# ProjectTorreyPines/TorJ.jl

Measured on AMD Instinct MI355X. Metric: ray-steps/sec, 1e5-ray EC fan on 1 MI355X (+ 2/4/8-GPU scaling), higher is better.
Workload: dtype f64

## Files before the change

### torj.jl_amd/csrc/torj_args.hpp

```cpp
#pragma once
#include "torj_math.hpp"

struct TraceArgs {
    const double *coef;
    const double *cellp;
    Grid g;
    Consts k;
    double omega;
    int mode;
    double ds;
    int n_steps;
    int chunk_steps;
    double psi_exit;
    double P_min;
    int n;
    const double *x0;
    const double *N0;
    const double *w;
    double *state;
    int *status;
    int *steps;
    int n_psi;
    const double *grid;
    double *dP;
// ... 11 lines not shown
    double abstol, reltol, s_step;
    int n_chunks;
    int *chunk;
    int n_hist, hist_off;
};

constexpr int kTsLds = 7 * 7 * 64;

constexpr int kDepoNone = 0, kDepoBinned = 1, kDepoSamples = 2;

#ifndef TORJ_BLOCK
#define TORJ_BLOCK 256
#endif
#ifndef TORJ_MIN_WAVES
#define TORJ_MIN_WAVES 2
#endif
#ifndef TORJ_GROUP
#define TORJ_GROUP 64
#endif
#ifndef TORJ_WARM_MIN_WAVES
#define TORJ_WARM_MIN_WAVES 1
#endif

constexpr int kAinF = 5;
constexpr int kAinFW = 6;

struct SplitArgs {
    double *ain;
    double *alpha;
    unsigned *awork;
    double *psib;
    double *cbx;
    double *tx;
    int *tinfo;
    double *stau, *spsi, *sPdep;
    int *sinfo;
    unsigned char *zflag;
    double zval;
    int k0, kb;
    int nf;
    int tile_cap;
    double tile_margin;
    int traj_mode;
    int nan_step;
    unsigned long long *defer;
    unsigned *defer_cnt;
    int defer_lrm;
    int zlatch;
};

constexpr int kSplitMaxSteps = 1 << 24;
__device__ __forceinline__ int info_steps(int v) { return v & 0xffffff; }
__device__ __forceinline__ int info_status(int v) { return (unsigned)v >> 24; }
__device__ __forceinline__ int make_info(int steps, int st) { return steps | (st << 24); }

#ifndef TORJ_AIN_TRAJ_MATH
#define TORJ_AIN_TRAJ_MATH 0
#endif
#ifndef TORJ_TRAJ_WAVES
#define TORJ_TRAJ_WAVES TORJ_MIN_WAVES
#endif
#ifndef TORJ_ALPHA_WAVES
#define TORJ_ALPHA_WAVES 6
#endif
#ifndef TORJ_ALPHA_UNROLL
#define TORJ_ALPHA_UNROLL 1
#endif
#ifndef TORJ_TILE_NODES
#define TORJ_TILE_NODES 256
#endif
constexpr int kTileNodes = TORJ_TILE_NODES;
#ifndef TORJ_TILE_CELLS
// ... 39 lines not shown
```

### torj.jl_amd/csrc/torj_k_alpha.hpp

```cpp
#pragma once
#include "torj_args.hpp"
#include "torj_k_fused.hpp"
#include "torj_warm.hpp"

#ifndef TORJ_ALPHA_BLOCK
#define TORJ_ALPHA_BLOCK 128
#endif
constexpr int kAlphaBlock = TORJ_ALPHA_BLOCK;
#ifndef TORJ_ALPHA_SETPRIO
#define TORJ_ALPHA_SETPRIO 0
#endif
template <bool COUNT>
__global__ void __launch_bounds__(kAlphaBlock, TORJ_ALPHA_WAVES) k_alpha_pts(TraceArgs a, SplitArgs sp, int nq) {
#if TORJ_ALPHA_SETPRIO
    __builtin_amdgcn_s_setprio(TORJ_ALPHA_SETPRIO);
#endif
    const int q = blockIdx.x, js = blockIdx.y;
    const int i = q * kAlphaBlock + threadIdx.x;
    if (i >= a.n) return;
    const int j = js >> 2;
    const int ti = sp.tinfo[i], si = sp.sinfo[i];
    const int zf = sp.zflag ? sp.zflag[i] : 0;
    if (__all(zf != 0)) {
#if defined(TORJ_ALPHA_PROF) && defined(__HIP_DEVICE_COMPILE__)
        TORJ_APROF_WAVE(kAprofZ);
#endif
        sp.alpha[(size_t)js * a.n + i] = sp.zval;
        if constexpr (COUNT) sp.awork[(size_t)js * a.n + i] = 0u;
        return;
    }
    const double *in = sp.ain + (size_t)js * sp.nf * a.n + i;
    const double X = in[0], Y = in[(size_t)a.n], N2 = in[2 * (size_t)a.n], Npar = in[3 * (size_t)a.n];
    const double lnTe = in[4 * (size_t)a.n];
    asm volatile("" ::"v"(ti), "v"(si), "v"(X), "v"(Y), "v"(N2), "v"(Npar), "v"(lnTe));
    if (sp.k0 + j >= info_steps(ti) || info_status(si) != ST_OK) return;
#if defined(TORJ_ALPHA_PROF) && defined(__HIP_DEVICE_COMPILE__)
    {
        const unsigned long long am = __ballot(1), zm = __ballot(zf != 0);
        if ((int)__lane_id() == __builtin_ffsll((long long)am) - 1) {
            atomicAdd(&g_aprof[4], 1ull);
            atomicAdd(&g_aprof[5], (unsigned long long)__popcll(am));
            atomicAdd(&g_aprof[14], (unsigned long long)__popcll(zm));
        }
    }
#endif
    const double Nabs = TORJ_AIN_TRAJ_MATH ? N2 : sqrt_pos(N2), Te = TORJ_AIN_TRAJ_MATH ? lnTe : exp_fast<true>(lnTe);
    if constexpr (COUNT) {
        AlbajarWork work = {};
        sp.alpha[(size_t)js * a.n + i] = abs_albajar_fast_body<1, TORJ_ALPHA_UNROLL>(
            c_gl, a.omega, X, Y, Nabs, Npar, Te, a.mode, &work, 0, c_gl.tiny_alpha);
        sp.awork[(size_t)js * a.n + i] = (work.n_active & 1u) | ((work.n_harm & 3u) << 1) |
                                     ((work.n_zero & 3u) << 3) | (min(work.n_terms, 2047u) << 5) |
                                     ((work.n_negl & 3u) << 16) | ((work.n_early & 3u) << 18);
    } else {
        sp.alpha[(size_t)js * a.n + i] = abs_albajar_fast_body<1, TORJ_ALPHA_UNROLL>(
            c_gl, a.omega, X, Y, Nabs, Npar, Te, a.mode, nullptr, 0, c_gl.tiny_alpha);
    }
}

#ifndef TORJ_ALPHA_PPW
#define TORJ_ALPHA_PPW 1
#endif
#ifndef TORJ_ALPHA_PREFETCH
#define TORJ_ALPHA_PREFETCH 1
#endif
template <bool COUNT, int P>
__global__ void __launch_bounds__(kAlphaBlock, TORJ_ALPHA_WAVES) k_alpha_pts_mp(TraceArgs a, SplitArgs sp, int nq) {
    const int i = blockIdx.x * kAlphaBlock + threadIdx.x;
    if (i >= a.n) return;
    const int js0 = blockIdx.y * P;
    const int np = min(P, 4 * sp.kb - js0);
    const int ti = sp.tinfo[i], si = sp.sinfo[i];
    const int js_end = info_status(si) != ST_OK ? 0 : 4 * (info_steps(ti) - sp.k0);
    const size_t n = (size_t)a.n, stride = (size_t)sp.nf * n;
    const double *in = sp.ain + (size_t)js0 * stride + i;
    double X = in[0], Y = in[n], N2 = in[2 * n], Npar = in[3 * n], lnTe = in[4 * n];
    for (int p = 0; p < np; p++) {
        const int js = js0 + p;
        const GLTable *glp = &c_gl;
        asm volatile("" : "+s"(glp));
#if TORJ_ALPHA_PREFETCH
        double Xn = 0.0, Yn = 0.0, N2n = 0.0, Nparn = 0.0, lnTen = 0.0;
        if (p + 1 < np) {
            const double *nx = in + (size_t)(p + 1) * stride;
            Xn = nx[0], Yn = nx[n], N2n = nx[2 * n], Nparn = nx[3 * n], lnTen = nx[4 * n];
        }
#endif
        if (js < js_end) {
            const double Nabs = TORJ_AIN_TRAJ_MATH ? N2 : sqrt_pos(N2),
                         Te = TORJ_AIN_TRAJ_MATH ? lnTe : exp_fast<true>(lnTe);
            if constexpr (COUNT) {
// ... 96 lines not shown
```

### torj.jl_amd/csrc/torj_k_scan.hpp

```cpp
#pragma once
#include "torj_args.hpp"
#include "torj_k_fused.hpp"
#include "torj_k_traj.hpp"

__device__ void cold_replay(const TraceArgs &a, const SplitArgs &sp, int i, double x[3], double N[3], int k) {
    const TileCell cg{a.cellp, nullptr, 0, 0, 0, 0};
    const TileCoef ng{a.coef, nullptr, 0, 0, 0, 0};
    ZBox zb;
    for (int s = 0; s < k; s++) {
        double xn[3], Nn[3], psi;
        double *o_run = ain_row(a, sp, 0, i);
        if (sp.traj_mode == kTrajCell)
            cold_step<true, kTileNS, TileCell, true>(a, cg, sp, 0, i, x, N, xn, Nn, &psi, zb, false, o_run);
        else if (sp.traj_mode == kTrajTile)
            cold_step<true, kTileNS, TileCoef, true>(a, ng, sp, 0, i, x, N, xn, Nn, &psi, zb, false, o_run);
        else
            cold_step<true, kNF, const double *, true>(a, a.coef, sp, 0, i, x, N, xn, Nn, &psi, zb, false, o_run);
#pragma unroll
        for (int c = 0; c < 3; c++) {
            x[c] = xn[c];
            N[c] = Nn[c];
        }
    }
}

template <int DEPO, bool TRAJ, bool COUNT>
__device__ __forceinline__ void tau_scan_body(const TraceArgs &a, const SplitArgs &sp) {
    const int i = blockIdx.x * 64 + threadIdx.x;
    unsigned long long nsteps = 0, c2 = 0, c3 = 0, c4 = 0, c5 = 0, c6 = 0, c7 = 0;
    const int am = a.abs_model;
    if (i < a.n) {
        int steps = 0, st = ST_OK;
        double tau = 0.0, psi_a = 0.0, Pdep = 0.0;
        if (sp.k0 > 0) {
            const int v = sp.sinfo[i];
            steps = info_steps(v);
            st = info_status(v);
            tau = sp.stau[i];
            Pdep = sp.sPdep[i];
        }
        if constexpr (DEPO == kDepoBinned) psi_a = sp.spsi[i];
        if (st == ST_OK) {
            const int tv = sp.tinfo[i];
            const int tT = info_steps(tv), tS = info_status(tv);
            const double w = (DEPO == kDepoBinned && a.w) ? a.w[i] : 1.0;
            const double ds6 = a.ds / 6.0;
            double P = exp(-tau);
            DepoAcc dacc = {-1, 0.0};
            const int s_end = min(a.n_steps, sp.k0 + sp.kb);
            constexpr int kScanBatch = 4;
            bool done = false;
            for (int sb = steps; sb < s_end && !done; sb += kScanBatch) {
                double alb[kScanBatch][4];
#pragma unroll
                for (int v = 0; v < kScanBatch; v++) {
                    const size_t ov = (size_t)(min(sb + v, s_end - 1) - sp.k0) * 4 * a.n + i;
#pragma unroll
                    for (int q = 0; q < 4; q++) alb[v][q] = sp.alpha[ov + q * (size_t)a.n];
                }
#pragma unroll
                for (int v = 0; v < kScanBatch; v++) {
                    const int s = sb + v;
                    if (s >= s_end) break;
                    if (s >= tT) {
                        if (tS == ST_NAN) st = ST_NAN;
                        done = true;
                        break;
                    }
                    const size_t o = (size_t)(s - sp.k0) * 4 * a.n + i;
                    const double al0 = (s == sp.nan_step && i % 3 == 0) ? (double)NAN : alb[v][0];
                    const double al1 = alb[v][1], al2 = alb[v][2], al3 = alb[v][3];
                    double acc_a = fma(1.0, al0, 0.0);
                    acc_a = fma(2.0, al1, acc_a);
                    acc_a = fma(2.0, al2, acc_a);
                    acc_a = fma(1.0, al3, acc_a);
                    const double taun = tau + ds6 * acc_a;
                    if (!isfinite(taun)) {
                        st = ST_NAN | 0x40;
                        done = true;
                        break;
                    }
#pragma unroll
                    for (int q = 0; q < 4 && COUNT; q++) {
                        const unsigned wk = sp.awork[o + q * (size_t)a.n];
                        if (am == 1) {
                            c2 += wk & 1u;
                            c3 += (wk >> 1) & 3u;
                            c5 += (wk >> 3) & 3u;
                            c4 += (wk >> 5) & 2047u;
                            c6 += (wk >> 16) & 3u;
                            c7 += (wk >> 18) & 3u;
                        } else if (am == 2) {
                            const unsigned lrm = wk >> 21, passes = (wk >> 14) & 127u;
                            c2 += wk & 127u;
                            c3 += (wk >> 7) & 127u;
                            c4 += passes;
                            c5 += passes * lrm;
                            c6 += lrm;
                            c7 += lrm * lrm;
                        }
                    }
                    const double Pn = exp(-taun);
                    const double dP = P - Pn;
                    if constexpr (DEPO == kDepoSamples) {
                        if (s > 0) a.smp_dpds[smp_at(s, i, a.smp_rows)] = P * al0;
                    }
                    tau = taun;
// ... 104 lines not shown
```

### torj.jl_amd/csrc/torj_k_traj.hpp

```cpp
#pragma once
#include "torj_args.hpp"
#include "torj_fitdepo.hpp"


#ifndef TORJ_TRAJ_AIN_STEP
#define TORJ_TRAJ_AIN_STEP 1
#endif
__device__ __forceinline__ double *ain_row(const TraceArgs &a, const SplitArgs &sp, int row, int i) {
    return sp.ain + ((size_t)row * sp.nf) * a.n + i;
}
template <bool STORE, int NS = kNF, class CS = const double *, bool PSI = false>
__device__ __forceinline__ bool cold_step(const TraceArgs &a, CS coef,
                                          const SplitArgs &sp, int j, int i, const double x[3],
                                          const double N[3], double xn[3], double Nn[3],
                                          double *psi_x, ZBox &zb, bool zon, double *&o_run) {
    const double hds = 0.5 * a.ds, ds6 = a.ds / 6.0;
    double acc[6] = {0, 0, 0, 0, 0, 0}, xt[3], Nt[3], k[6];
#pragma unroll
    for (int c = 0; c < 3; c++) {
        xt[c] = x[c];
        Nt[c] = N[c];
    }
    constexpr bool kCellTrim = IsTileCell<CS>::value;
#pragma unroll 1
// ... 156 lines not shown
                cb[c * (size_t)a.n] = x[c];
                cb[(3 + c) * (size_t)a.n] = N[c];
            }
        }
        if (zlatch && zon) {
            trips++;
            if (trips == kZLatchTrip0 || trips == kZLatchTrip1) {
                if (!__any(zero_box_flag(zb))) {
                    zero_box_kill(zb);
                    zon = false;
                }
            }
        }
    }
    double invR;
    if (pending && step_end(steps - 1, eval_one<NS>(coef, a.g, cyl_radius(x, invR), x[2], F_PSI)))
        st = ST_LEFT_PLASMA;
#pragma unroll
    for (int c = 0; c < 3; c++) {
        sp.tx[c * (size_t)a.n + i] = x[c];
        sp.tx[(3 + c) * (size_t)a.n + i] = N[c];
    }
    sp.tinfo[i] = make_info(steps, st);
    if (sp.zflag != nullptr) sp.zflag[i] = zero_box_flag(zb) ? 1 : 0;
}


template <int DEPO, bool TRAJ, int MODE>
__device__ __forceinline__ void traj_body(const TraceArgs &a, const SplitArgs &sp) {
    const int i = blockIdx.x * blockDim.x + threadIdx.x;
    double x[3] = {0, 0, 0}, N[3] = {0, 0, 0};
    int steps = 0, st = ST_OK;
    bool live = i < a.n;
    if (live) {
        if (sp.k0 == 0) {
#pragma unroll
            for (int c = 0; c < 3; c++) {
                x[c] = a.x0[c * a.n + i];
                N[c] = a.N0[c * a.n + i];
                sp.cbx[c * (size_t)a.n + i] = x[c];
                sp.cbx[(3 + c) * (size_t)a.n + i] = N[c];
            }
        } else {
            const int v = sp.tinfo[i];
            steps = info_steps(v);
            st = info_status(v);
#pragma unroll
            for (int c = 0; c < 3; c++) {
                x[c] = sp.tx[c * (size_t)a.n + i];
                N[c] = sp.tx[(3 + c) * (size_t)a.n + i];
            }
        }
        live = st == ST_OK && !(sp.k0 > 0 && info_status(sp.sinfo[i]) != ST_OK);
        if (!live && sp.zflag) sp.zflag[i] = 1;
    }
    if constexpr (MODE == kTrajTile) {
        __shared__ __attribute__((aligned(16))) double s_tile[kTileNodes * kTileNS];
        const double R = sqrt(x[0] * x[0] + x[1] * x[1]);
        const double inf = __builtin_inf();
        const double rmin = wave_min(live ? R : inf), rmax = wave_max(live ? R : -inf);
        const double zmin = wave_min(live ? x[2] : inf), zmax = wave_max(live ? x[2] : -inf);
        if (!(rmin <= rmax && zmin <= zmax)) return;
        const double m = (double)(sp.kb + 1) * a.ds * sp.tile_margin;
        const int iR0 = cell_index(rmin - m, a.g.R1, a.g.Rn, a.g.invhR, a.g.nR),
                  iR1 = cell_index(rmax + m, a.g.R1, a.g.Rn, a.g.invhR, a.g.nR),
                  iZ0 = cell_index(zmin - m, a.g.Z1, a.g.Zn, a.g.invhZ, a.g.nZ),
                  iZ1 = cell_index(zmax + m, a.g.Z1, a.g.Zn, a.g.invhZ, a.g.nZ);
        TileCoef tc{a.coef, s_tile, iR0, iZ0, iR1 - iR0 + 4, iZ1 - iZ0 + 4};
        if (tc.tw * tc.th > sp.tile_cap) {
            tc.tw = tc.th = 0;
        } else {
            const int mR = a.g.nR + 2, cnt = tc.tw * tc.th * kTileNS;
            for (int k = threadIdx.x; k < cnt; k += 64) {
                const int node = k / kTileNS, f = k - node * kTileNS;
                const int zr = node / tc.tw, rr = node - zr * tc.tw;
                s_tile[k] = a.coef[((size_t)(iZ0 + zr) * mR + iR0 + rr) * kNF + f];
            }
        }
        __syncthreads();
        if (!live) return;
        traj_run<DEPO, TRAJ, kTileNS>(a, sp, tc, i, x, N, steps, st);
    } else if constexpr (MODE == kTrajCell) {
        __shared__ __attribute__((aligned(16))) double s_cell[kTileCells * kCellRec];
        const double R = sqrt(x[0] * x[0] + x[1] * x[1]);
        const double inf = __builtin_inf();
        const double rmin = wave_min(live ? R : inf), rmax = wave_max(live ? R : -inf);
        const double zmin = wave_min(live ? x[2] : inf), zmax = wave_max(live ? x[2] : -inf);
        if (!(rmin <= rmax && zmin <= zmax)) return;
        const double m = (double)(sp.kb + 1) * a.ds * sp.tile_margin;
        const int iR0 = cell_index(rmin - m, a.g.R1, a.g.Rn, a.g.invhR, a.g.nR),
                  iR1 = cell_index(rmax + m, a.g.R1, a.g.Rn, a.g.invhR, a.g.nR),
                  iZ0 = cell_index(zmin - m, a.g.Z1, a.g.Zn, a.g.invhZ, a.g.nZ),
                  iZ1 = cell_index(zmax + m, a.g.Z1, a.g.Zn, a.g.invhZ, a.g.nZ);
        const int cR0 = __builtin_amdgcn_readfirstlane(iR0), cZ0 = __builtin_amdgcn_readfirstlane(iZ0);
        const int cw = __builtin_amdgcn_readfirstlane(iR1 - iR0 + 1), ch = __builtin_amdgcn_readfirstlane(iZ1 - iZ0 + 1);
        TileCell tc{a.cellp, s_cell, cR0, cZ0, cw, ch};
        if (cw * ch > sp.tile_cap) {
            tc.cw = tc.ch = 0;
        } else {
            const int cR = a.g.nR - 1;
            const Dbl2 *src = reinterpret_cast<const Dbl2 *>(a.cellp);
            Dbl2 *dst = reinterpret_cast<Dbl2 *>(s_cell);
            for (int zr = 0; zr < ch; zr++)
                for (int rr = 0; rr < cw; rr++)
                    if (threadIdx.x < kCellRec / 2)
                        dst[(zr * cw + rr) * (kCellRec / 2) + threadIdx.x] =
                            src[((size_t)(cZ0 + zr) * cR + cR0 + rr) * (kCellRec / 2) + threadIdx.x];
        }
        __syncthreads();
        if (!live) return;
        traj_run<DEPO, TRAJ, kTileNS>(a, sp, tc, i, x, N, steps, st);
    } else if constexpr (MODE == kTrajLds) {
        extern __shared__ __attribute__((aligned(16))) double s_coef[];
        const int nodes = (a.g.nR + 2) * (a.g.nZ + 2);
        for (int k = threadIdx.x; k < nodes * kTrajLdsNS; k += blockDim.x)
            s_coef[k] = a.coef[(size_t)(k / kTrajLdsNS) * kNF + k % kTrajLdsNS];
        __syncthreads();
        if (!live) return;
        traj_run<DEPO, TRAJ, kTrajLdsNS>(a, sp, (const double *)s_coef, i, x, N, steps, st);
    } else {
        if (!live) return;
        traj_run<DEPO, TRAJ, kNF>(a, sp, (const double *)a.coef, i, x, N, steps, st);
    }
}

template <int DEPO, bool TRAJ>
__global__ void __launch_bounds__(64, TORJ_TRAJ_WAVES) k_traj(TraceArgs a, SplitArgs sp) {
    traj_body<DEPO, TRAJ, kTrajL2>(a, sp);
}
// ... 26 lines not shown
```

### torj.jl_amd/csrc/torj_math.hpp

```cpp
#pragma once

#include <hip/hip_runtime.h>
#include <math.h>
#include <stdint.h>

#include "torj_bessel_coefs.hpp"

#define TORJ_HD __host__ __device__ __forceinline__

namespace torj {

constexpr double kC = 2.99792458e8;
constexpr double kE = 1.602176634e-19;
constexpr double kMe = 9.1093837015e-31;
constexpr double kEps0 = 8.8541878128e-12;
constexpr double kPi = 3.14159265358979323846;

constexpr int kNF = 8;
enum Field { F_BR = 0, F_BPHI = 1, F_BZ = 2, F_LNNE = 3, F_LNTE = 4, F_PSI = 5 };

enum Status { ST_OK = 0, ST_LEFT_PLASMA = 1, ST_ABSORBED = 2, ST_NAN = 3, ST_REFLECTED = 4,
              ST_ENTRY_FAIL = 5, ST_MAX_STEPS = 6 };

struct Grid {
// ... 331 lines not shown
    for (int f = 0; f < NT; f++) {
        const double gR = PHYS ? gr[f] : gr[f] * g.invhR, gZ = PHYS ? gz[f] : gz[f] * g.invhZ;
        if constexpr (EXT) {
            out.v[f] = v[f] + dRx * gR + dZx * gZ;
        } else {
            out.v[f] = v[f];
        }
        if (f < NGRAD) {
            const int q = f < NGRAD ? f : 0;
            if constexpr (EXT) {
                const double gRZ = PHYS ? grz[f] : grz[f] * (g.invhR * g.invhZ);
                out.dR[q] = outR ? gR : gR + dZx * gRZ;
                out.dZ[q] = outZ ? gZ : gZ + dRx * gRZ;
            } else {
                out.dR[q] = gR;
                out.dZ[q] = gZ;
            }
        }
    }
}

constexpr int kCellNS = 6;
constexpr int kCellRec = kCellNS * 16;
struct CellAxis {
    int i;
    double t, delta;
};
#ifndef TORJ_CELL_AXIS_FAST
#define TORJ_CELL_AXIS_FAST 1
#endif
#if defined(__HIP_DEVICE_COMPILE__) && TORJ_CELL_AXIS_FAST
constexpr bool kCellAxisFast = true;
#else
constexpr bool kCellAxisFast = false;
#endif
TORJ_HD void cell_axis(double x, double x1, double xn, double h, double invh, int n, CellAxis &a) {
#if defined(__HIP_DEVICE_COMPILE__) && TORJ_CELL_AXIS_FAST
    asm("" : "+v"(x));
    double xc;
    asm("v_max_f64 %0, %1, %2" : "=v"(xc) : "v"(x), "s"(x1));
    asm("v_min_f64 %0, %1, %2" : "=v"(xc) : "v"(xc), "s"(xn));
    a.delta = x - xc;
    const double u = (xc - x1) * invh;
    int i;
    asm("v_med3_i32 %0, %1, 0, %2" : "=v"(i) : "v"((int)u), "s"(n - 2));
    a.t = (u - (double)i) * h;
// ... 49 lines not shown
        for (int k = 0; k < 8; k++) A[k] = reinterpret_cast<Q>(c + fidx[f] * 16)[k];
        cell_field(A, tR, tZ, EXT || f < NGRAD, EXT && f < NGRAD, v[f], gr[f], gz[f], grz[f]);
    }
}
template <int NGRAD, int NVAL, bool EXT = true, int NS = kNF>
TORJ_HD void eval_fields(const TileCell &t, const Grid &g, const CellAxis &aR, const CellAxis &aZ,
                         const int (&fidx)[NGRAD + NVAL], FieldPack<NGRAD, NVAL> &out) {
    constexpr int NT = NGRAD + NVAL;
    const int dR = aR.i - t.cR0, dZ = aZ.i - t.cZ0;
    bool in = kCellAxisFast ? (unsigned)dR < (unsigned)t.cw && (unsigned)dZ < (unsigned)t.ch
                            : dR >= 0 && dR < t.cw && dZ >= 0 && dZ < t.ch;
#ifdef __HIP_DEVICE_COMPILE__
    in = __all(in);
    using LdsP = const __attribute__((address_space(3))) double *;
    using GlbP = const __attribute__((address_space(1))) double *;
#else
    using LdsP = const double *;
    using GlbP = const double *;
#endif
    double v[NT], gr[NT], gz[NT], grz[NT];
#pragma unroll
    for (int f = 0; f < NT; f++) gr[f] = gz[f] = grz[f] = 0.0;
    if (in)
        cell_sums<NGRAD, NVAL, EXT, LdsP>((LdsP)t.lds + (size_t)(dZ * t.cw + dR) * kCellRec, aR, aZ, fidx, v,
                                          gr, gz, grz);
    else
        cell_sums<NGRAD, NVAL, EXT, GlbP>((GlbP)t.g + ((size_t)aZ.i * (g.nR - 1) + aR.i) * kCellRec, aR, aZ,
                                          fidx, v, gr, gz, grz);
    fields_finish_d<NGRAD, NVAL, EXT, true>(g, aR.delta, aZ.delta, v, gr, gz, grz, out);
}
template <int NGRAD, int NVAL, bool EXT = true, int NS = kNF>
TORJ_HD void eval_fields(const TileCell &t, const Grid &g, double R, double Z,
                         const int (&fidx)[NGRAD + NVAL], FieldPack<NGRAD, NVAL> &out) {
    CellAxis aR, aZ;
    cell_axis(R, g.R1, g.Rn, g.hR, g.invhR, g.nR, aR);
    cell_axis(Z, g.Z1, g.Zn, g.hZ, g.invhZ, g.nZ, aZ);
    eval_fields<NGRAD, NVAL, EXT, NS>(t, g, aR, aZ, fidx, out);
}
inline void cell_power_table(const double *coef, int nR, int nZ, double hR, double hZ, double *out) {
    const long double s6 = 1.0L / 6.0L;
    const long double B[4][4] = {{s6, 4 * s6, s6, 0.0L},
                                 {-0.5L, 0.0L, 0.5L, 0.0L},
                                 {0.5L, -1.0L, 0.5L, 0.0L},
                                 {-s6, 0.5L, -0.5L, s6}};
    const int mR = nR + 2;
    for (int iZ = 0; iZ < nZ - 1; iZ++)
        for (int iR = 0; iR < nR - 1; iR++)
// ... 914 lines not shown
```

### torj.jl_amd/csrc/torj_plasma.hpp

```cpp
#pragma once
#include <rccl/rccl.h>

#include <algorithm>
#include <mutex>
#include <vector>

#include "torj_host_util.hpp"
#include "torj_math.hpp"

static void bspl1d_prefilter(int n, const double *y, size_t ystride, double *c, size_t cstride) {
    auto C = [&](int k) -> double & { return c[(size_t)k * cstride]; };
    auto Y = [&](int k) { return y[(size_t)k * ystride]; };
    C(1) = Y(0);
    C(n) = Y(n - 1);
    const int m = n - 2;
    if (m > 0) {
        std::vector<double> cp(m), dp(m);
        for (int k = 0; k < m; k++) {
            double r = 6.0 * Y(k + 1);
            if (k == 0) r -= C(1);
            if (k == m - 1) r -= C(n);
            const double den = 4.0 - (k > 0 ? cp[k - 1] : 0.0);
            cp[k] = 1.0 / den;
            dp[k] = (r - (k > 0 ? dp[k - 1] : 0.0)) / den;
        }
        C(m + 1) = dp[m - 1];
        for (int k = m - 2; k >= 0; k--) C(k + 2) = dp[k] - cp[k] * C(k + 3);
    }
    C(0) = 2.0 * C(1) - C(2);
// ... 94 lines not shown
    GrowBuf batch;
    std::vector<hipEvent_t> ev_pool;
    size_t ev_used = 0;
    GrowBuf ws;
    GrowBuf beams;
    int *d_flags = nullptr;
    int n_cu = 256;
    std::mutex mu;
    std::vector<torj_plasma_s *> replicas;
    std::vector<ncclComm_t> comms;
    struct BeamStage {
        void *d = nullptr, *h = nullptr;
        size_t d_cap = 0, h_cap = 0;
        bool h_pinned = false;
        hipStream_t sc = nullptr;
        hipEvent_t up[2] = {}, tr[2] = {}, dn[2] = {};
    } stage;
    double reduce_ms = 0.0;
    int reduce_calls = 0;
    GrowBuf split;
    hipStream_t stream2 = nullptr, streamT = nullptr;
    hipStream_t streamS = nullptr;
    hipStream_t streamD = nullptr;
    static constexpr int kRing = 4;
    hipEvent_t ev_T[kRing] = {}, ev_A[kRing] = {}, ev_S[kRing] = {}, ev_J = nullptr, ev_F = nullptr;
    hipEvent_t ev_D = nullptr;
    hipEvent_t ev_Nin = nullptr, ev_Nout = nullptr;
};

static const int kFieldSlot[6] = {F_PSI, F_LNNE, F_LNTE, F_BR, F_BZ, F_BPHI};

static int plasma_finish(torj_plasma_s *p, int nR, int nZ, double R1, double Rn, double Z1,
                         double Zn, const double *const fields[6], int device,
                         torj_plasma_t *out) {
    p->device = device;
    Grid &g = p->g;
    g.nR = nR;
    g.nZ = nZ;
    g.R1 = R1;
    g.Rn = Rn;
    g.Z1 = Z1;
    g.Zn = Zn;
    g.hR = (Rn - R1) / (nR - 1);
    g.hZ = (Zn - Z1) / (nZ - 1);
    g.invhR = 1.0 / g.hR;
    g.invhZ = 1.0 / g.hZ;
    const size_t nodes = (size_t)(nR + 2) * (nZ + 2);
// ... 111 lines not shown
```

### torj.jl_amd/csrc/torj_split.hpp

```cpp
#pragma once
#include <atomic>

#include "torj_dispatch.hpp"
#include "torj_k_alpha.hpp"
#include "torj_k_depo.hpp"
#include "torj_k_scan.hpp"
#include "torj_k_traj.hpp"
#include "torj_plasma.hpp"

static size_t fit_grid_lds(int n_psi) { return n_psi <= kFitGridLds ? (size_t)n_psi * sizeof(double) : 0; }

static int fit_zero(const FitArgs &fa, hipStream_t st) {
    const size_t L = (size_t)fa.n_psi, N = (size_t)fa.n;
    HIPCK(hipMemsetAsync(fa.cnt, 0, (L + 1) * N * sizeof(int), st));
    HIPCK(hipMemsetAsync(fa.Fopen, 0xFF, L * N * sizeof(double), st));
    HIPCK(hipMemsetAsync(fa.dPs, 0, L * N * sizeof(double), st));
    return 0;
}

struct SplitPlan {
    static constexpr int R = torj_plasma_s::kRing;
    size_t n;
    int n_steps, nf;
    long kb, first;
    int n_blk;
    size_t b_ain, b_alpha, b_awork, b_psib, b_cbx, b_n8, b_n4, b_zf, b_dsd, b_dsi, b_defer, b_dcnt, bytes;
    bool zflag_on, dstream, serial;
    int dstream_env, depo_lag, lds_env, tile_cap, nan_step, zflag_nan_from, defer_lrm, zlatch;
    double tile_margin;

    int block_k0(int b) const { return (int)(first ? (b == 0 ? 0 : first + (long)(b - 1) * kb) : b * kb); }
    int block_len(int b) const { return (int)std::min<long>(first && b == 0 ? first : kb, n_steps - block_k0(b)); }
    int window_cap(int bw) const {
        return (int)(first ? (bw == 0 ? first : first + (long)bw * kb) : std::min<long>((long)(bw + 1) * kb, n_steps));
    }
};

static int split_plan(SplitPlan &pl, const torj_plasma_s *p, const TraceArgs &a, int DM, bool walk,
                      bool negl_skip) {
    const size_t n = pl.n = (size_t)a.n;
    const int n_steps = pl.n_steps = a.n_steps;
    static const size_t budget_env = (size_t)env_long("TORJ_SPLIT_MB", 1024) << 20;
    size_t free_b = 0, total_b = 0;
    HIPCK(hipMemGetInfo(&free_b, &total_b));
    const size_t budget = std::max<size_t>(std::min(budget_env, free_b / 16), 1);
    pl.nf = a.abs_model >= 2 ? kAinFW : kAinF;
    const size_t per_step = 4 * (size_t)pl.nf * sizeof(double) * n;
    long kb = (long)std::max<size_t>(1, budget / per_step);
    kb = std::min<long>(kb, 16383);
    if (a.chunk_steps > 0 && kb >= a.chunk_steps) kb -= kb % a.chunk_steps;
    if (p->sched_mode == 3 && p->sched_waves > 0) kb = std::min(p->sched_waves, 16383);
    kb = pl.kb = std::min<long>(kb, n_steps);
    const int n_cb = (a.chunk_steps > 0 ? n_steps / a.chunk_steps : 0) + 1;
    auto al = [](size_t b) { return (b + 255) & ~(size_t)255; };
    pl.b_ain = al(per_step * kb);
    pl.b_alpha = al(4 * sizeof(double) * n * kb);
    pl.b_awork = a.counters ? al(4 * sizeof(unsigned) * n * kb) : 0;
    pl.b_psib = DM == kDepoBinned ? al(sizeof(double) * n * kb) : 0;
    pl.b_cbx = al(6 * sizeof(double) * n * n_cb);
    pl.b_n8 = al(8 * n);
    pl.b_n4 = al(4 * n);
    pl.zflag_on = a.abs_model == 1 && negl_skip && env_int("TORJ_ALPHA_ZFLAG", 1) != 0;
    pl.b_zf = pl.zflag_on ? al(n) : 0;
    pl.zlatch = env_int("TORJ_ZBOX_LATCH", 1) != 0;
    pl.dstream_env = env_int("TORJ_DEPO_STREAM", 3);
    pl.dstream = walk && pl.dstream_env != 0;
    pl.b_dsd = pl.dstream ? al(kDsNd * sizeof(double) * n) : 0;
    pl.b_dsi = pl.dstream ? al(kDsNi * sizeof(int) * n) : 0;
    long first = env_long("TORJ_SPLIT_FIRST", 0);
    if (a.chunk_steps > 0 && first > 0) first = std::max<long>(a.chunk_steps, first - first % a.chunk_steps);
    if (first >= kb || first >= n_steps) first = 0;
    pl.first = first;
    pl.n_blk = first ? 1 + (int)((n_steps - first + kb - 1) / kb) : (int)((n_steps + kb - 1) / kb);
    pl.b_defer = a.abs_model >= 2 ? al(4 * sizeof(unsigned long long) * n * kb) : 0;
    pl.b_dcnt = a.abs_model >= 2 ? al(sizeof(unsigned) * pl.n_blk) : 0;
    pl.bytes = pl.R * (pl.b_ain + pl.b_alpha + pl.b_awork) + pl.R * pl.b_psib + pl.b_cbx + 6 * pl.b_n8 +
               3 * pl.b_n8 + 2 * pl.b_n4 + pl.b_dsd + pl.b_dsi + pl.b_defer + pl.b_dcnt + pl.R * pl.b_zf;
    pl.serial = env_int("TORJ_SPLIT_SERIAL", 0) != 0;
    pl.depo_lag = std::min(torj_plasma_s::kRing - 1, std::max(1, env_int("TORJ_DEPO_LAG", 2)));
    pl.lds_env = env_int("TORJ_TRAJ_LDS", 3);
    const int tile_max = pl.lds_env == 3 ? kTileCells : kTileNodes;
    pl.tile_cap = std::min(tile_max, env_int("TORJ_TILE_CAP", tile_max));
    pl.tile_margin = env_double("TORJ_TILE_MARGIN", 1.001);
    pl.nan_step = env_int("TORJ_TEST_NAN_ALPHA_STEP", -1);
    if (pl.nan_step >= 0) {
        static std::atomic<bool> warned{false};
        if (!warned.exchange(true))
            fprintf(stderr, "libtorj_hip: TORJ_TEST_NAN_ALPHA_STEP=%d is set -- a TEST HOOK: alpha is "
                            "read as NaN at that step for every third ray\n", pl.nan_step);
    }
    pl.zflag_nan_from = env_has("TORJ_TEST_ZFLAG_NAN") ? std::max(0, env_int("TORJ_TEST_ZFLAG_NAN", 0)) : -1;
    if (pl.zflag_nan_from >= 0) {
        static std::atomic<bool> warned{false};
        if (!warned.exchange(true))
            fprintf(stderr, "libtorj_hip: TORJ_TEST_ZFLAG_NAN is set -- a TEST HOOK: fully flagged alpha "
                            "waves write NaN\n");
    }
    pl.defer_lrm = std::min(3, std::max(0, env_int("TORJ_WARM_DEFER_LRM", 3)));
    return 0;
}

struct SplitRing {
    static constexpr int R = SplitPlan::R;
    double *ain[R], *alphas[R], *psib[R];
    unsigned *aworks[R];
    unsigned char *zflags[R];
    unsigned *dcnt;
    DepoStream ds;
};

static void split_carve(const SplitPlan &pl, char *q, SplitArgs &sp, SplitRing &rg) {
    constexpr int R = SplitPlan::R;
    auto take = [&](size_t b) {
        char *r = q;
        q += b;
        return r;
    };
    rg = SplitRing{};
    for (int r = 0; r < R; r++) rg.ain[r] = (double *)take(pl.b_ain);
    for (int r = 0; r < R; r++) {
        rg.alphas[r] = (double *)take(pl.b_alpha);
        rg.aworks[r] = (unsigned *)take(pl.b_awork);
    }
    if (pl.b_psib)
        for (int r = 0; r < R; r++) rg.psib[r] = (double *)take(pl.b_psib);
    if (pl.b_zf)
        for (int r = 0; r < R; r++) rg.zflags[r] = (unsigned char *)take(pl.b_zf);
    sp.cbx = (double *)take(pl.b_cbx);
    sp.tx = (double *)take(6 * pl.b_n8);
    sp.stau = (double *)take(pl.b_n8);
    sp.spsi = (double *)take(pl.b_n8);
    sp.sPdep = (double *)take(pl.b_n8);
    sp.tinfo = (int *)take(pl.b_n4);
    sp.sinfo = (int *)take(pl.b_n4);
    sp.defer = pl.b_defer ? (unsigned long long *)take(pl.b_defer) : nullptr;
    rg.dcnt = pl.b_dcnt ? (unsigned *)take(pl.b_dcnt) : nullptr;
    if (pl.dstream) {
        rg.ds.d = (double *)take(pl.b_dsd);
        rg.ds.v = (int *)take(pl.b_dsi);
    }
}

static int split_trace(torj_plasma_s *p, TraceArgs a, int DM, bool tr, hipStream_t s, const FitArgs *fa,
                       DepoStream *dso, bool negl_skip) {
    SplitPlan pl;
    if (split_plan(pl, p, a, DM, fa && dso, negl_skip)) return -1;
    constexpr int R = SplitPlan::R;
    const size_t n = pl.n;
    if (ensure_split(p, pl.bytes)) return -1;
    SplitArgs sp{};
    SplitRing rg;
    split_carve(pl, (char *)p->split.d, sp, rg);
    const DepoStream ds = rg.ds;
    if (dso) *dso = ds;
    sp.nf = pl.nf;
    sp.tile_cap = pl.tile_cap;
    sp.tile_margin = pl.tile_margin;
    sp.nan_step = pl.nan_step;
    sp.zval = 0.0;
    sp.defer_lrm = pl.defer_lrm;
    sp.zlatch = pl.zlatch;

    const bool serial = pl.serial, dstream = pl.dstream;
// ... 18 lines not shown
    HIPCK(hipMemsetAsync(sp.sinfo, 0, pl.b_n4, sT));
    if (dstream) HIPCK(hipMemsetAsync(ds.v + kDsJ * n, 0xFF, n * sizeof(int), sT));
    if (rg.dcnt) HIPCK(hipMemsetAsync(rg.dcnt, 0, pl.n_blk * sizeof(unsigned), s2));
    if (fa && fit_zero(*fa, s3)) return -1;
    const size_t fit_lds = fa ? fit_grid_lds(fa->n_psi) : 0;
    const int G = (int)((n + 63) / 64);
    const size_t lds_bytes = (size_t)(a.g.nR + 2) * (a.g.nZ + 2) * kTrajLdsNS * sizeof(double);
    const bool lds_traj = pl.lds_env == 1 && lds_bytes <= 160 * 1024;
    const bool tile_traj = pl.lds_env == 2, cell_traj = pl.lds_env == 3;
    sp.traj_mode = cell_traj ? kTrajCell : tile_traj ? kTrajTile : lds_traj ? kTrajLds : kTrajL2;
    const int wpb = std::min(8, std::max(1, (G + p->n_cu - 1) / p->n_cu));
    const int n_blocks = pl.n_blk;
    auto depo_pair = [&](hipStream_t st, int cap) {
        hipLaunchKernelGGL(k_depo_elim, dim3(G), dim3(64), 0, st, *fa, ds, sp.sinfo, cap);
        hipLaunchKernelGGL(k_depo_walk, dim3(G), dim3(64), fit_lds, st, *fa, ds, sp.sinfo, cap);
    };
    for (int b = 0; b < n_blocks; b++) {
        sp.k0 = pl.block_k0(b);
        sp.kb = pl.block_len(b);
        const int r = b % R;
        sp.ain = rg.ain[r];
        sp.psib = rg.psib[r];
        sp.zflag = rg.zflags[r];
        sp.zval = (pl.zflag_nan_from >= 0 && sp.k0 >= pl.zflag_nan_from) ? NAN : 0.0;
        sp.alpha = rg.alphas[r];
        sp.awork = pl.b_awork ? rg.aworks[r] : nullptr;
        if (b >= R) HIPCK(hipStreamWaitEvent(sT, p->ev_S[r], 0));
        if (depo_traj && b >= pl.depo_lag) {
            const int bw = b - pl.depo_lag;
            HIPCK(hipStreamWaitEvent(sT, p->ev_S[bw % R], 0));
            depo_pair(sT, pl.window_cap(bw));
        }
        with_depo_traj(DM, tr, [&](auto D, auto T) {
            if (cell_traj)
                hipLaunchKernelGGL((k_traj_cell<D(), T()>), dim3(G), dim3(64), 0, sT, a, sp);
            else if (tile_traj)
                hipLaunchKernelGGL((k_traj_tile<D(), T()>), dim3(G), dim3(64), 0, sT, a, sp);
            else if (lds_traj)
                hipLaunchKernelGGL((k_traj_lds<D(), T()>), dim3(nblocks(G, wpb)), dim3(64 * wpb), lds_bytes, sT, a, sp);
            else
                hipLaunchKernelGGL((k_traj<D(), T()>), dim3(G), dim3(64), 0, sT, a, sp);
        });
        HIPCK(hipEventRecord(p->ev_T[r], sT));
        HIPCK(hipStreamWaitEvent(s2, p->ev_T[r], 0));
        const int nqA = (int)((n + kAlphaBlock - 1) / kAlphaBlock);
        const dim3 agridA((unsigned)nqA, (unsigned)(4 * sp.kb));
// ... 46 lines not shown
            }
        }
    }
    if (depo_traj) {
        for (int bw = std::max(0, n_blocks - pl.depo_lag); bw + 1 < n_blocks; bw++) {
            HIPCK(hipStreamWaitEvent(sT, p->ev_S[bw % R], 0));
            depo_pair(sT, pl.window_cap(bw));
        }
    }
    with_depo_traj(DM, tr, [&](auto D, auto T) {
        hipLaunchKernelGGL((k_split_final<D(), T()>), dim3(G), dim3(64), 0, s3, a, sp);
    });
    if (!serial) {
        HIPCK(hipEventRecord(p->ev_J, s3));
        HIPCK(hipStreamWaitEvent(s, p->ev_J, 0));
        if (depo_own || depo_traj) {
            HIPCK(hipEventRecord(p->ev_D, depo_traj ? sT : sD));
            HIPCK(hipStreamWaitEvent(s, p->ev_D, 0));
        }
    }
    HIPCK(hipGetLastError());
    return 0;
}
```

Before: 5.758 billion.

## Add per-wave group zero flags so alpha and scan skip all-zero ray groups

The trajectory kernels now write a per-64-ray group flag marking waves whose rays are all dead or all inside the zero-absorption box. The alpha kernels read this flag through a scalar constant-address load and exit the whole wave before touching per-ray inputs or writing alpha. The scan kernel substitutes zval and zero work counts for flagged groups instead of reading the alpha and awork buffers. This cuts memory traffic and launch work for fully inactive waves, at the cost of a small ring-buffered flag array and an extra wave vote in the trajectory kernel. The change also adds an optional LDS padding for cell records (off by default) and splits the plan sizing into its own host function.

```diff
diff --git a/torj.jl_amd/csrc/torj_args.hpp b/torj.jl_amd/csrc/torj_args.hpp
--- a/torj.jl_amd/csrc/torj_args.hpp
+++ b/torj.jl_amd/csrc/torj_args.hpp
@@ -57,6 +57,8 @@
 #define TORJ_WARM_MIN_WAVES 1
 #endif
 
+constexpr int kSplitRing = 4;
+
 constexpr int kAinF = 5;
 constexpr int kAinFW = 6;
 
@@ -72,6 +74,7 @@
     int *sinfo;
     unsigned char *zflag;
     double zval;
+    unsigned *gflag;
     int k0, kb;
     int nf;
     int tile_cap;
@@ -83,6 +86,15 @@
     int defer_lrm;
     int zlatch;
 };
+
+__device__ __forceinline__ unsigned group_word(const unsigned *gflag, int g) {
+#if defined(__HIP_DEVICE_COMPILE__)
+    typedef const __attribute__((address_space(4))) unsigned *const_ptr;
+    return ((const_ptr)(unsigned long long)gflag)[g];
+#else
+    return gflag[g];
+#endif
+}
 
 constexpr int kSplitMaxSteps = 1 << 24;
 __device__ __forceinline__ int info_steps(int v) { return v & 0xffffff; }
diff --git a/torj.jl_amd/csrc/torj_k_alpha.hpp b/torj.jl_amd/csrc/torj_k_alpha.hpp
--- a/torj.jl_amd/csrc/torj_k_alpha.hpp
+++ b/torj.jl_amd/csrc/torj_k_alpha.hpp
@@ -7,6 +7,19 @@
 #define TORJ_ALPHA_BLOCK 128
 #endif
 constexpr int kAlphaBlock = TORJ_ALPHA_BLOCK;
+static_assert(kAlphaBlock % 64 == 0, "an alpha wave holds one 64-ray group");
+#if defined(__HIP_DEVICE_COMPILE__)
+#define TORJ_ALPHA_ARGS_BATCH(a, sp)                                                                        \
+    asm volatile("" ::"s"((a).n), "s"((sp).gflag), "s"((sp).zflag), "s"((sp).tinfo), "s"((sp).sinfo),      \
+                 "s"((sp).ain), "s"((sp).alpha), "s"((sp).nf), "s"((sp).k0))
+#else
+#define TORJ_ALPHA_ARGS_BATCH(a, sp) \
+    do {                             \
+    } while (0)
+#endif
+__device__ __forceinline__ bool alpha_group_flagged(const SplitArgs &sp, int w0) {
+    return sp.gflag != nullptr && group_word(sp.gflag, w0 >> 6) != 0u;
+}
 #ifndef TORJ_ALPHA_SETPRIO
 #define TORJ_ALPHA_SETPRIO 0
 #endif
@@ -17,11 +30,29 @@
 #endif
     const int q = blockIdx.x, js = blockIdx.y;
     const int i = q * kAlphaBlock + threadIdx.x;
+    TORJ_ALPHA_ARGS_BATCH(a, sp);
+    const int w0 = __builtin_amdgcn_readfirstlane(i & ~63);
+    if (w0 >= a.n) return;
+    if (alpha_group_flagged(sp, w0)) {
+#if defined(TORJ_ALPHA_PROF) && defined(__HIP_DEVICE_COMPILE__)
+        TORJ_APROF_WAVE(kAprofZ);
+#endif
+        return;
+    }
     if (i >= a.n) return;
     const int j = js >> 2;
+#if defined(TORJ_ALPHA_PROF)
+    const bool want_zf = sp.zflag != nullptr;
+#else
+    const bool want_zf = sp.zflag != nullptr && sp.gflag == nullptr;
+#endif
     const int ti = sp.tinfo[i], si = sp.sinfo[i];
-    const int zf = sp.zflag ? sp.zflag[i] : 0;
-    if (__all(zf != 0)) {
+    const int zf = want_zf ? sp.zflag[i] : 0;
+    const double *in = sp.ain + (size_t)js * sp.nf * a.n + i;
+    const double X = in[0], Y = in[(size_t)a.n], N2 = in[2 * (size_t)a.n], Npar = in[3 * (size_t)a.n];
+    const double lnTe = in[4 * (size_t)a.n];
+    asm volatile("" ::"v"(ti), "v"(si), "v"(zf), "v"(X), "v"(Y), "v"(N2), "v"(Npar), "v"(lnTe));
+    if (sp.gflag == nullptr && __all(zf != 0)) {
 #if defined(TORJ_ALPHA_PROF) && defined(__HIP_DEVICE_COMPILE__)
         TORJ_APROF_WAVE(kAprofZ);
 #endif
@@ -29,10 +60,6 @@
         if constexpr (COUNT) sp.awork[(size_t)js * a.n + i] = 0u;
         return;
     }
-    const double *in = sp.ain + (size_t)js * sp.nf * a.n + i;
-    const double X = in[0], Y = in[(size_t)a.n], N2 = in[2 * (size_t)a.n], Npar = in[3 * (size_t)a.n];
-    const double lnTe = in[4 * (size_t)a.n];
-    asm volatile("" ::"v"(ti), "v"(si), "v"(X), "v"(Y), "v"(N2), "v"(Npar), "v"(lnTe));
     if (sp.k0 + j >= info_steps(ti) || info_status(si) != ST_OK) return;
 #if defined(TORJ_ALPHA_PROF) && defined(__HIP_DEVICE_COMPILE__)
     {
@@ -67,6 +94,10 @@
 template <bool COUNT, int P>
 __global__ void __launch_bounds__(kAlphaBlock, TORJ_ALPHA_WAVES) k_alpha_pts_mp(TraceArgs a, SplitArgs sp, int nq) {
     const int i = blockIdx.x * kAlphaBlock + threadIdx.x;
+    TORJ_ALPHA_ARGS_BATCH(a, sp);
+    const int w0 = __builtin_amdgcn_readfirstlane(i & ~63);
+    if (w0 >= a.n) return;
+    if (alpha_group_flagged(sp, w0)) return;
     if (i >= a.n) return;
     const int js0 = blockIdx.y * P;
     const int np = min(P, 4 * sp.kb - js0);
diff --git a/torj.jl_amd/csrc/torj_k_scan.hpp b/torj.jl_amd/csrc/torj_k_scan.hpp
--- a/torj.jl_amd/csrc/torj_k_scan.hpp
+++ b/torj.jl_amd/csrc/torj_k_scan.hpp
@@ -29,19 +29,24 @@
     const int i = blockIdx.x * 64 + threadIdx.x;
     unsigned long long nsteps = 0, c2 = 0, c3 = 0, c4 = 0, c5 = 0, c6 = 0, c7 = 0;
     const int am = a.abs_model;
+    const bool gz = sp.gflag != nullptr && group_word(sp.gflag, (int)blockIdx.x) != 0u;
     if (i < a.n) {
         int steps = 0, st = ST_OK;
         double tau = 0.0, psi_a = 0.0, Pdep = 0.0;
+        int sv = 0;
+        const int tv = sp.tinfo[i];
         if (sp.k0 > 0) {
-            const int v = sp.sinfo[i];
-            steps = info_steps(v);
-            st = info_status(v);
+            sv = sp.sinfo[i];
             tau = sp.stau[i];
             Pdep = sp.sPdep[i];
         }
         if constexpr (DEPO == kDepoBinned) psi_a = sp.spsi[i];
+#if defined(__HIP_DEVICE_COMPILE__)
+        asm volatile("" ::"v"(tv), "v"(sv), "v"(tau), "v"(Pdep), "v"(psi_a));
+#endif
+        steps = info_steps(sv);
+        st = info_status(sv);
         if (st == ST_OK) {
-            const int tv = sp.tinfo[i];
             const int tT = info_steps(tv), tS = info_status(tv);
             const double w = (DEPO == kDepoBinned && a.w) ? a.w[i] : 1.0;
             const double ds6 = a.ds / 6.0;
@@ -56,7 +61,7 @@
                 for (int v = 0; v < kScanBatch; v++) {
                     const size_t ov = (size_t)(min(sb + v, s_end - 1) - sp.k0) * 4 * a.n + i;
 #pragma unroll
-                    for (int q = 0; q < 4; q++) alb[v][q] = sp.alpha[ov + q * (size_t)a.n];
+                    for (int q = 0; q < 4; q++) alb[v][q] = gz ? sp.zval : sp.alpha[ov + q * (size_t)a.n];
                 }
 #pragma unroll
                 for (int v = 0; v < kScanBatch; v++) {
@@ -82,7 +87,7 @@
                     }
 #pragma unroll
                     for (int q = 0; q < 4 && COUNT; q++) {
-                        const unsigned wk = sp.awork[o + q * (size_t)a.n];
+                        const unsigned wk = gz ? 0u : sp.awork[o + q * (size_t)a.n];
                         if (am == 1) {
                             c2 += wk & 1u;
                             c3 += (wk >> 1) & 3u;
diff --git a/torj.jl_amd/csrc/torj_k_traj.hpp b/torj.jl_amd/csrc/torj_k_traj.hpp
--- a/torj.jl_amd/csrc/torj_k_traj.hpp
+++ b/torj.jl_amd/csrc/torj_k_traj.hpp
@@ -202,7 +202,11 @@
         sp.tx[(3 + c) * (size_t)a.n + i] = N[c];
     }
     sp.tinfo[i] = make_info(steps, st);
-    if (sp.zflag != nullptr) sp.zflag[i] = zero_box_flag(zb) ? 1 : 0;
+    if (sp.zflag != nullptr) {
+        const bool zf = zero_box_flag(zb);
+        sp.zflag[i] = zf ? 1 : 0;
+        if (sp.gflag != nullptr) sp.gflag[i >> 6] = __all(zf) ? 1u : 0u;
+    }
 }
 
 
@@ -234,6 +238,7 @@
         live = st == ST_OK && !(sp.k0 > 0 && info_status(sp.sinfo[i]) != ST_OK);
         if (!live && sp.zflag) sp.zflag[i] = 1;
     }
+    if (sp.gflag != nullptr && !__any(live) && i < a.n) sp.gflag[i >> 6] = 1u;
     if constexpr (MODE == kTrajTile) {
         __shared__ __attribute__((aligned(16))) double s_tile[kTileNodes * kTileNS];
         const double R = sqrt(x[0] * x[0] + x[1] * x[1]);
@@ -261,7 +266,7 @@
         if (!live) return;
         traj_run<DEPO, TRAJ, kTileNS>(a, sp, tc, i, x, N, steps, st);
     } else if constexpr (MODE == kTrajCell) {
-        __shared__ __attribute__((aligned(16))) double s_cell[kTileCells * kCellRec];
+        __shared__ __attribute__((aligned(16))) double s_cell[kTileCells * kCellLds];
         const double R = sqrt(x[0] * x[0] + x[1] * x[1]);
         const double inf = __builtin_inf();
         const double rmin = wave_min(live ? R : inf), rmax = wave_max(live ? R : -inf);
@@ -284,7 +289,7 @@
             for (int zr = 0; zr < ch; zr++)
                 for (int rr = 0; rr < cw; rr++)
                     if (threadIdx.x < kCellRec / 2)
-                        dst[(zr * cw + rr) * (kCellRec / 2) + threadIdx.x] =
+                        dst[(zr * cw + rr) * (kCellLds / 2) + threadIdx.x] =
                             src[((size_t)(cZ0 + zr) * cR + cR0 + rr) * (kCellRec / 2) + threadIdx.x];
         }
         __syncthreads();
diff --git a/torj.jl_amd/csrc/torj_math.hpp b/torj.jl_amd/csrc/torj_math.hpp
--- a/torj.jl_amd/csrc/torj_math.hpp
+++ b/torj.jl_amd/csrc/torj_math.hpp
@@ -377,6 +377,10 @@
 
 constexpr int kCellNS = 6;
 constexpr int kCellRec = kCellNS * 16;
+#ifndef TORJ_CELL_LDS_PAD
+#define TORJ_CELL_LDS_PAD 0
+#endif
+constexpr int kCellLds = kCellRec + (TORJ_CELL_LDS_PAD ? 2 : 0);
 struct CellAxis {
     int i;
     double t, delta;
@@ -472,7 +476,7 @@
 #pragma unroll
     for (int f = 0; f < NT; f++) gr[f] = gz[f] = grz[f] = 0.0;
     if (in)
-        cell_sums<NGRAD, NVAL, EXT, LdsP>((LdsP)t.lds + (size_t)(dZ * t.cw + dR) * kCellRec, aR, aZ, fidx, v,
+        cell_sums<NGRAD, NVAL, EXT, LdsP>((LdsP)t.lds + (size_t)(dZ * t.cw + dR) * kCellLds, aR, aZ, fidx, v,
                                           gr, gz, grz);
     else
         cell_sums<NGRAD, NVAL, EXT, GlbP>((GlbP)t.g + ((size_t)aZ.i * (g.nR - 1) + aR.i) * kCellRec, aR, aZ,
diff --git a/torj.jl_amd/csrc/torj_plasma.hpp b/torj.jl_amd/csrc/torj_plasma.hpp
--- a/torj.jl_amd/csrc/torj_plasma.hpp
+++ b/torj.jl_amd/csrc/torj_plasma.hpp
@@ -5,6 +5,7 @@
 #include <mutex>
 #include <vector>
 
+#include "torj_args.hpp"
 #include "torj_host_util.hpp"
 #include "torj_math.hpp"
 
@@ -145,7 +146,7 @@
     hipStream_t stream2 = nullptr, streamT = nullptr;
     hipStream_t streamS = nullptr;
     hipStream_t streamD = nullptr;
-    static constexpr int kRing = 4;
+    static constexpr int kRing = kSplitRing;
     hipEvent_t ev_T[kRing] = {}, ev_A[kRing] = {}, ev_S[kRing] = {}, ev_J = nullptr, ev_F = nullptr;
     hipEvent_t ev_D = nullptr;
     hipEvent_t ev_Nin = nullptr, ev_Nout = nullptr;
diff --git a/torj.jl_amd/csrc/torj_split.hpp b/torj.jl_amd/csrc/torj_split.hpp
--- a/torj.jl_amd/csrc/torj_split.hpp
+++ b/torj.jl_amd/csrc/torj_split.hpp
@@ -1,6 +1,11 @@
 #pragma once
+#include <algorithm>
 #include <atomic>
 
+#include "torj_args.hpp"
+#include "torj_fitdepo.hpp"
+#include "torj_host_util.hpp"
+#ifndef TORJ_SPLIT_PLAN_ONLY
 #include "torj_dispatch.hpp"
 #include "torj_k_alpha.hpp"
 #include "torj_k_depo.hpp"
@@ -17,15 +22,16 @@
     HIPCK(hipMemsetAsync(fa.dPs, 0, L * N * sizeof(double), st));
     return 0;
 }
+#endif
 
 struct SplitPlan {
-    static constexpr int R = torj_plasma_s::kRing;
+    static constexpr int R = kSplitRing;
     size_t n;
     int n_steps, nf;
     long kb, first;
     int n_blk;
-    size_t b_ain, b_alpha, b_awork, b_psib, b_cbx, b_n8, b_n4, b_zf, b_dsd, b_dsi, b_defer, b_dcnt, bytes;
-    bool zflag_on, dstream, serial;
+    size_t b_ain, b_alpha, b_awork, b_psib, b_cbx, b_n8, b_n4, b_zf, b_gf, b_dsd, b_dsi, b_defer, b_dcnt, bytes;
+    bool zflag_on, gflag_on, dstream, serial;
     int dstream_env, depo_lag, lds_env, tile_cap, nan_step, zflag_nan_from, defer_lrm, zlatch;
     double tile_margin;
 
@@ -36,20 +42,18 @@
     }
 };
 
-static int split_plan(SplitPlan &pl, const torj_plasma_s *p, const TraceArgs &a, int DM, bool walk,
-                      bool negl_skip) {
+static void split_plan_sizes(SplitPlan &pl, int sched_mode, int sched_waves, size_t free_b, const TraceArgs &a,
+                             int DM, bool walk, bool negl_skip) {
     const size_t n = pl.n = (size_t)a.n;
     const int n_steps = pl.n_steps = a.n_steps;
     static const size_t budget_env = (size_t)env_long("TORJ_SPLIT_MB", 1024) << 20;
-    size_t free_b = 0, total_b = 0;
-    HIPCK(hipMemGetInfo(&free_b, &total_b));
     const size_t budget = std::max<size_t>(std::min(budget_env, free_b / 16), 1);
     pl.nf = a.abs_model >= 2 ? kAinFW : kAinF;
     const size_t per_step = 4 * (size_t)pl.nf * sizeof(double) * n;
     long kb = (long)std::max<size_t>(1, budget / per_step);
     kb = std::min<long>(kb, 16383);
     if (a.chunk_steps > 0 && kb >= a.chunk_steps) kb -= kb % a.chunk_steps;
-    if (p->sched_mode == 3 && p->sched_waves > 0) kb = std::min(p->sched_waves, 16383);
+    if (sched_mode == 3 && sched_waves > 0) kb = std::min(sched_waves, 16383);
     kb = pl.kb = std::min<long>(kb, n_steps);
     const int n_cb = (a.chunk_steps > 0 ? n_steps / a.chunk_steps : 0) + 1;
     auto al = [](size_t b) { return (b + 255) & ~(size_t)255; };
@@ -62,6 +66,8 @@
     pl.b_n4 = al(4 * n);
     pl.zflag_on = a.abs_model == 1 && negl_skip && env_int("TORJ_ALPHA_ZFLAG", 1) != 0;
     pl.b_zf = pl.zflag_on ? al(n) : 0;
+    pl.gflag_on = pl.zflag_on && env_int("TORJ_ALPHA_GFLAG", 1) != 0;
+    pl.b_gf = pl.gflag_on ? al(sizeof(unsigned) * ((n + 63) / 64)) : 0;
     pl.zlatch = env_int("TORJ_ZBOX_LATCH", 1) != 0;
     pl.dstream_env = env_int("TORJ_DEPO_STREAM", 3);
     pl.dstream = walk && pl.dstream_env != 0;
@@ -75,9 +81,9 @@
     pl.b_defer = a.abs_model >= 2 ? al(4 * sizeof(unsigned long long) * n * kb) : 0;
     pl.b_dcnt = a.abs_model >= 2 ? al(sizeof(unsigned) * pl.n_blk) : 0;
     pl.bytes = pl.R * (pl.b_ain + pl.b_alpha + pl.b_awork) + pl.R * pl.b_psib + pl.b_cbx + 6 * pl.b_n8 +
-               3 * pl.b_n8 + 2 * pl.b_n4 + pl.b_dsd + pl.b_dsi + pl.b_defer + pl.b_dcnt + pl.R * pl.b_zf;
+               3 * pl.b_n8 + 2 * pl.b_n4 + pl.b_dsd + pl.b_dsi + pl.b_defer + pl.b_dcnt + pl.R * pl.b_zf + pl.R * pl.b_gf;
     pl.serial = env_int("TORJ_SPLIT_SERIAL", 0) != 0;
-    pl.depo_lag = std::min(torj_plasma_s::kRing - 1, std::max(1, env_int("TORJ_DEPO_LAG", 2)));
+    pl.depo_lag = std::min(kSplitRing - 1, std::max(1, env_int("TORJ_DEPO_LAG", 2)));
     pl.lds_env = env_int("TORJ_TRAJ_LDS", 3);
     const int tile_max = pl.lds_env == 3 ? kTileCells : kTileNodes;
     pl.tile_cap = std::min(tile_max, env_int("TORJ_TILE_CAP", tile_max));
@@ -97,7 +103,6 @@
                             "waves write NaN\n");
     }
     pl.defer_lrm = std::min(3, std::max(0, env_int("TORJ_WARM_DEFER_LRM", 3)));
-    return 0;
 }
 
 struct SplitRing {
@@ -105,6 +110,7 @@
     double *ain[R], *alphas[R], *psib[R];
     unsigned *aworks[R];
     unsigned char *zflags[R];
+    unsigned *gflags[R];
     unsigned *dcnt;
     DepoStream ds;
 };
@@ -126,6 +132,8 @@
         for (int r = 0; r < R; r++) rg.psib[r] = (double *)take(pl.b_psib);
     if (pl.b_zf)
         for (int r = 0; r < R; r++) rg.zflags[r] = (unsigned char *)take(pl.b_zf);
+    if (pl.b_gf)
+        for (int r = 0; r < R; r++) rg.gflags[r] = (unsigned *)take(pl.b_gf);
     sp.cbx = (double *)take(pl.b_cbx);
     sp.tx = (double *)take(6 * pl.b_n8);
     sp.stau = (double *)take(pl.b_n8);
@@ -139,6 +147,15 @@
         rg.ds.d = (double *)take(pl.b_dsd);
         rg.ds.v = (int *)take(pl.b_dsi);
     }
+}
+
+#ifndef TORJ_SPLIT_PLAN_ONLY
+static int split_plan(SplitPlan &pl, const torj_plasma_s *p, const TraceArgs &a, int DM, bool walk,
+                      bool negl_skip) {
+    size_t free_b = 0, total_b = 0;
+    HIPCK(hipMemGetInfo(&free_b, &total_b));
+    split_plan_sizes(pl, p->sched_mode, p->sched_waves, free_b, a, DM, walk, negl_skip);
+    return 0;
 }
 
 static int split_trace(torj_plasma_s *p, TraceArgs a, int DM, bool tr, hipStream_t s, const FitArgs *fa,
@@ -203,6 +220,7 @@
         sp.ain = rg.ain[r];
         sp.psib = rg.psib[r];
         sp.zflag = rg.zflags[r];
+        sp.gflag = rg.gflags[r];
         sp.zval = (pl.zflag_nan_from >= 0 && sp.k0 >= pl.zflag_nan_from) ? NAN : 0.0;
         sp.alpha = rg.alphas[r];
         sp.awork = pl.b_awork ? rg.aworks[r] : nullptr;
@@ -295,3 +313,4 @@
     HIPCK(hipGetLastError());
     return 0;
 }
+#endif
```

Result: faster. 5.865 billion, median of 6 (+1.9%).
